# jmduarte/gnn-fpga

Hardware: AMD Instinct MI355X
Metric: edges/sec (EdgeNet+NodeNet fwd) on 100k-edge TrackML graphs; % HBM roofline (higher is better)
Workload: dtype f32; 1 GPU; c3 synthetic TrackML ACTS graphs: 256 graphs/launch/GPU x (10k hits, 100k segments), F=3, D=8, 3 MP iterations + final edge pass, index form resident in HBM; graphs_per_gpu=256, hits_per_graph=10000, segments_per_graph=100000

## Files before the change

### gnn-fpga_amd/csrc/sell_pipeline.hip

```cpp
#include "common.h"

#include <cstdlib>
#include <type_traits>

namespace {
using namespace gnn;

constexpr int SLICE = 16;
constexpr int DESC = 8;

template <int F, int D>
struct TL {
    static constexpr int d4 = D / 4, C = F + D;
    static constexpr int a4(int x) { return (x + 3) & ~3; }
    static constexpr int o_w2 = 0;
    static constexpr int o_in = a4(o_w2 + d4);
    static constexpr int in_sz = d4 + F * d4;
    static constexpr int o_4 = a4(o_in + in_sz);
    static constexpr int w4_sz = d4 + D * d4;
    static constexpr int o_m = a4(o_4 + w4_sz);
    static constexpr int m_sz = d4 + C * d4;
    static constexpr int m_st = a4(m_sz);
    static constexpr int o_b2 = o_m + 5 * m_st;
    static constexpr int used = o_b2 + 1;
// ... 1839 lines not shown
        }
        const int nq = (sg1 - sg0 + NTEAM - 1) / NTEAM;
        const int q0 = (((local - rot) % per_xcd) + per_xcd) % per_xcd;
        rot = (rot + nq) % per_xcd;
        for (int q = q0; SPLIT && sg0 + NTEAM * q < sg1; q += per_xcd) {
            const int sl = sg0 + NTEAM * q + team;
            if (sl >= sg1) continue;
            const int ib = __builtin_amdgcn_readfirstlane(in_off[sl]);
            const int il = (__builtin_amdgcn_readfirstlane(in_off[sl + 1]) - ib) >> 4;
            if (il <= 0) continue;
            const int i16 = 4 * mem + hs;
            const int64_t n = (int64_t)sl * SLICE + i16;
            float acc[DL], ownQ[DL];
            load_vec<DL>(U + n * D + DL * p, acc);
            load_own_w<D, EX>(QS, n, p, ownQ);
            sweep_w<D, XP, EX>(in_nbr + ib, i16, il, (int)n_pad, PR, p, ownQ, w2, b2, acc);
            store_vec<DL>(U + n * D + DL * p, acc);
        }
        if constexpr (SPLIT) {
            ++ngrp;
            if (lane == 0) bump(pha);
            for (int spins = 0; spins < kSpinLimit && ld(pha) < NSW * ngrp; ++spins) __builtin_amdgcn_s_sleep(2);
        }
        for (int q = q0; sg0 + NTEAM * q < sg1; q += per_xcd, seq += NTEAM) {
            const int sl = sg0 + NTEAM * q + team;
            const bool on = sl < sg1;
            float acc[DL];
            if (on) {
                const int ob = __builtin_amdgcn_readfirstlane(out_off[sl]);
                const int ol = (__builtin_amdgcn_readfirstlane(out_off[sl + 1]) - ob) >> 4;
                const int i16 = 4 * mem + hs;
                const int64_t n = (int64_t)sl * SLICE + i16;
                float ownP[DL];
                load_vec<DL>(U + n * D + DL * p, acc);
                if constexpr (!SPLIT) {
                    const int ib = __builtin_amdgcn_readfirstlane(in_off[sl]);
                    const int il = (__builtin_amdgcn_readfirstlane(in_off[sl + 1]) - ib) >> 4;
                    float ownQ[DL];
                    load_own_w<D, EX>(QS, n, p, ownQ);
                    load_own_w<D, EX>(PR, n, p, ownP);
                    sweep_w<D, XP, EX>(in_nbr + ib, i16, il, (int)n_pad, PR, p, ownQ, w2, b2, acc);
                } else {
                    load_own_w<D, EX>(PR, n, p, ownP);
                }
                sweep_w<D, XP, EX>(out_nbr + ob, i16, ol, (int)n_pad, QS, p, ownP, w2, b2, acc);
#pragma unroll
                for (int i = 0; i < DL; ++i) acc[i] = tanh_f(acc[i]);
            }
            const int slot = seq % NSLOT, gen = seq / NSLOT;
            for (int spins = 0; spins < kSpinLimit && ld(cons + slot) < gen; ++spins) __builtin_amdgcn_s_sleep(2);
            float *tr = ring + slot * 16 * B::tr_stride;
            if (on) {
                const int i16 = 4 * mem + hs;
                const int64_t n = (int64_t)sl * SLICE + i16;
                store_vec<DL>(tr + i16 * B::tr_stride + DL * p, acc);
                if (p < F) tr[i16 * B::tr_stride + D + p] = X[n * F + p];
            }
            if (mem == 0 && lane == 0) __hip_atomic_store(meta + slot, on ? sl : -1, __ATOMIC_RELAXED, __HIP_MEMORY_SCOPE_WORKGROUP);
            asm volatile("s_waitcnt lgkmcnt(0)" ::: "memory");
            if (lane == 0) bump(prod + slot);
        }
        if constexpr (!SPLIT) {
            ++ngrp;
            if (lane == 0) bump(pha);
            for (int spins = 0; spins < kSpinLimit && ld(pha) < NSW * ngrp; ++spins) __builtin_amdgcn_s_sleep(2);
        }
    }
    asm volatile("s_waitcnt lgkmcnt(0)" ::: "memory");
    if (lane == 0) bump(fin);
}

template <int F, int D>
struct MT {
    static_assert(D == 8, "fp32 matrix-core tables are laid out for D = 8");
    static constexpr int C = F + D;
    static constexpr bool PACK = F <= 4;
    static constexpr int NS = PACK ? 3 : F <= 8 ? 4 : 5;
    static constexpr int o_h0 = 0;
    static constexpr int o_t = 64;
    static constexpr int t_sz = NS * 64;
    static constexpr int o_w4 = o_t + 3 * t_sz;
    static constexpr int o_b = o_w4 + 128;
    static constexpr int total = o_b + 5 * 16;
    static constexpr int slot_k(int s, int g)
    {
        if (PACK) {
            if (g == 0) return s;
            if (g == 1) return 4 + s;
            if (g == 2) return s == 0 ? 3 : s == 1 ? 7 : (0 < F ? D : -1);
            return 1 + s < F ? D + 1 + s : -1;
        }
        if (s < 4) {
            if (g == 0) return s;
            if (g == 1) return 4 + s;
            const int xi = (g == 2) ? s : 4 + s;
            return xi < F ? D + xi : -1;
        }
        return 8 + g < F ? D + 8 + g : -1;
    }
};

template <int F, int D>
constexpr int mt_total()
{
    if constexpr (D == 8) return MT<F, D>::total;
    else return 0;
}

template <int F, int D>
__device__ __forceinline__ float mt_entry(const gnn_params_t &p, int i, bool last)
{
    using M = MT<F, D>;
    constexpr int C = F + D;
    if (i < 64) {
        const int row = i & 15, g = i >> 4;
        return (row < 8 && g < F && g < 4) ? p.Win[row * F + g] : 0.0f;
    }
    if (i < M::o_w4) {
        const int j = i - M::o_t, T = j / M::t_sz, st = (j % M::t_sz) >> 6, row = j & 15, g = (j >> 4) & 3;
        const int k = M::slot_k(st, g);
        if (k < 0) return 0.0f;
        if (last) {
            if (T > 0) return 0.0f;
            return kTwoLog2e * p.W1[(row & 7) * 2 * C + (row >> 3) * C + k];
        }
        if (T == 2) return row < 8 ? p.W3[row * 3 * C + 2 * C + k] : 0.0f;
        const int c = row >> 2, w = row & 3, d = 2 * c + (w & 1);
        return (w < 2) ? kTwoLog2e * p.W1[d * 2 * C + T * C + k] : p.W3[d * 3 * C + T * C + k];
    }
    if (i < M::o_b) {
        const int j = i - M::o_w4, st = j >> 6, row = j & 15, g = (j >> 4) & 3;
        return row < 8 ? p.W4[row * D + 2 * g + st] : 0.0f;
    }
    const int j = i - M::o_b, which = j >> 4, row = j & 15;
    switch (which) {
    case 0: return row < 8 ? p.bin[row] : 0.0f;
    case 1:
        if (last) return row < 8 ? kTwoLog2e * p.b1[row] : 0.0f;
        return (row & 3) < 2 ? kTwoLog2e * p.b1[2 * (row >> 2) + (row & 1)] : 0.0f;
    case 2: return 0.0f;
    case 3: return (!last && row < 8) ? p.b3[row] : 0.0f;
    default: return row < 8 ? p.b4[row] : 0.0f;
    }
}

template <int F, int D, bool LAST, bool XP, bool FIRST>
__global__ __launch_bounds__(1024) void k_iter2(
    const float *__restrict__ X, const float *__restrict__ table, gnn_params_t p,
    float *__restrict__ table_out,
    const int32_t *__restrict__ tiles, const int32_t *__restrict__ in_off,
    const int32_t *__restrict__ in_off16, const int32_t *__restrict__ in_nbr16,
    const int32_t *__restrict__ out_off, const int32_t *__restrict__ out_off16,
    const int32_t *__restrict__ out_nbr16, const int32_t *__restrict__ sched_a,
    const int32_t *__restrict__ sched_b, const float *__restrict__ PR,
    const float *__restrict__ QS, float *__restrict__ U, float *__restrict__ PRn,
    float *__restrict__ QSn, float *__restrict__ Pc, float *__restrict__ Qc, int64_t n_pad,
    int n_tiles, int capA, int capB, int xbuf_floats)
{
    using L = TL<F, D>;
    constexpr int d4 = L::d4, NT = 1024, NWV = NT / 64, NC = 3;
    extern __shared__ __attribute__((aligned(16))) float smem[];
    float *lds = smem, *bufA = smem + L::total, *bufB = bufA + (int64_t)capA * 2 * D;
    float *xbuf = bufB + (int64_t)capB * 2 * D;
    const int tid = threadIdx.x, lane = tid & 63, q = lane & 3, i16 = lane >> 2;
    const int wv = __builtin_amdgcn_readfirstlane(tid >> 6);
    if constexpr (FIRST) {
        for (int idx = tid; idx < L::total; idx += NT) {
            const float v = table_entry<F, D>(p, idx);
            lds[idx] = v;
            if (blockIdx.x == 0) table_out[idx] = v;
        }
        if (blockIdx.x == 0)
            write_null_rows<F, D, XP>(p, PRn, const_cast<float *>(PR), QSn, const_cast<float *>(QS),
                                      U, Pc, Qc, n_pad);
    } else {
        stage4<NT>(table, lds, L::total / 4);
    }
    float *mt = xbuf + (FIRST ? xbuf_floats : 0);
    if constexpr (D == 8)
        for (int i = tid; i < MT<F, D>::total; i += NT) mt[i] = mt_entry<F, D>(p, i, LAST);
    int tile = (gridDim.x & 7) ? (int)blockIdx.x
                               : (int)((blockIdx.x & 7) * (gridDim.x >> 3) + (blockIdx.x >> 3));
    if (tile >= n_tiles) return;

    struct Desc { int s_begin, s_end, in_lo, in_cnt, out_lo, out_cnt, sbase; };
    auto load_desc = [&](int t) {
        const int32_t *td = tiles + (int64_t)t * DESC;
        Desc d;
        d.s_begin = td[0]; d.s_end = td[1]; d.in_lo = td[2]; d.in_cnt = td[3];
        d.out_lo = td[4]; d.out_cnt = td[5]; d.sbase = td[7];
        return d;
    };
    auto slice_a = [&](const Desc &d, int r) { return sched_a[d.sbase + r * NWV + wv]; };

    auto stage_issue = [&](const float *src, float *buf, int nrec) {
        const int pieces = (nrec * 2 * D + 255) / 256;
        unsigned lb = (unsigned)lane * 16u;
        asm volatile("" : "+v"(lb));
        for (int c = wv; c < pieces; c += NWV)
            __builtin_amdgcn_global_load_lds(
                (const __attribute__((address_space(1))) void *)(
                    reinterpret_cast<const char *>(src + (int64_t)c * 256) + lb),
                (__attribute__((address_space(3))) void *)(buf + c * 256), 16, 0, 0);
    };
    auto put_null = [&](float *buf, int nrec, auto which) {
        constexpr int M = decltype(which)::value;
        const int pieces = (nrec * 2 * D + 255) / 256;
        if (wv == (pieces > 0 ? (pieces - 1) % NWV : 0) && lane < 4) {
            int l = lane;
            asm volatile("" : "+v"(l));
#pragma unroll
            for (int i = 0; i < d4; ++i) {
                float v = (M == 0) ? lds[l * L::stride + L::o_m + i] : 0.0f, z = 0.0f;
                if (XP) v = (M == 0) ? __builtin_amdgcn_exp2f(v) : 1.0f;
                asm volatile("" : "+v"(v), "+v"(z));
                buf[nrec * 2 * D + l * 2 * d4 + i] = v;
                buf[nrec * 2 * D + l * 2 * d4 + d4 + i] = z;
            }
        }
    };
    using WinA = std::integral_constant<int, 0>;
    using WinB = std::integral_constant<int, 1>;
    auto stage_commit = [&](float *buf, int nrec, auto which) {
        a_wait_all();
        put_null(buf, nrec, which);
    };

    auto x_image = [&](float *buf, int cap) { return buf + cap * 2 * D - (cap * F + 63) / 64 * 64; };
    auto xstage_issue = [&](int lo, int cnt, float *buf, int cap) {
        const int pieces = (cnt * F + 63) / 64;
        float *xb = x_image(buf, cap);
        unsigned lb = (unsigned)lane * 4u;
        asm volatile("" : "+v"(lb));
        for (int c = wv; c < pieces; c += NWV)
            __builtin_amdgcn_global_load_lds(
                (const __attribute__((address_space(1))) void *)(
                    reinterpret_cast<const char *>(X + (int64_t)lo * F + c * 64) + lb),
                (__attribute__((address_space(3))) void *)(xb + c * 64), 4, 0, 0);
    };
    auto h0_of = [&](const float *wl, const float *x, float *hn) {
        float hl[d4];
        role_gemv<d4, 0, F>(wl + L::o_in, x, x, hl);
#pragma unroll
        for (int i = 0; i < d4; ++i) hl[i] = tanh_f(hl[i]);
        quad_allgather<d4>(hl, hn);
    };
    auto compute_window = [&](float *buf, int cnt, int cap, auto which) {
        constexpr int M = decltype(which)::value;
        static_assert(2 * D * 4 - F * 4 >= 16, "a record must be longer than an X row (see x_image)");
        const float *xb = x_image(buf, cap);
        const int rounds = (cnt + NT / 4 - 1) / (NT / 4);
        const int x_off = (int)(xb - buf);
        auto round_fence = [&](int r) {
            if ((r + 1) * (NT / 4) * 2 * D > x_off) __syncthreads();
        };
        auto null_fence = [&]() {
            if ((cnt + 1) * 2 * D > x_off) __syncthreads();
        };
        a_wait_all();
        __syncthreads();
        if constexpr (D == 8) {
            typedef float f4v __attribute__((ext_vector_type(4)));
            using MTL = MT<F, D>;
            const float *mb = mt + MTL::o_b;
            const int hit = lane & 15, g = lane >> 4;
            const float a0 = mt[MTL::o_h0 + lane];
            static_assert(MTL::PACK, "the fused first launch exists for F <= 3 only");
            float ar[MTL::NS];
#pragma unroll
            for (int st = 0; st < MTL::NS; ++st) ar[st] = mt[MTL::o_t + MTL::t_sz * M + 64 * st + lane];
            const f4v bias0 = *reinterpret_cast<const f4v *>(mb + 4 * g);
            const f4v biasr = *reinterpret_cast<const f4v *>(mb + 16 + 16 * M + 4 * g);
            for (int r = 0; r < rounds; ++r) {
                const int h = (r * NWV + wv) * 16 + hit;
                const bool live = h < cnt;
                float xs[F];
#pragma unroll
                for (int k = 0; k < F; ++k) xs[k] = live ? xb[h * F + k] : 0.0f;
                round_fence(r);
                float b0 = 0.0f;
#pragma unroll
                for (int k = 0; k < F; ++k) b0 = (g == k) ? xs[k] : b0;
                f4v hq = __builtin_amdgcn_mfma_f32_16x16x4f32(a0, b0, bias0, 0, 0, 0);
                const float hh[4] = {tanh_f(hq.x), tanh_f(hq.y), tanh_f(hq.z), tanh_f(hq.w)};
                const float h3a = __int_as_float(__builtin_amdgcn_ds_bpermute(hit << 2, __float_as_int(hh[3])));
                const float h3b = __int_as_float(__builtin_amdgcn_ds_bpermute((16 + hit) << 2, __float_as_int(hh[3])));
                f4v c = biasr;
#pragma unroll
                for (int st = 0; st < MTL::NS; ++st) {
                    float b = hh[st];
                    if (g == 2) b = st == 0 ? h3a : st == 1 ? h3b : xs[0];
                    if (g == 3) b = 1 + st < F ? xs[1 + st < F ? 1 + st : 0] : 0.0f;
                    c = __builtin_amdgcn_mfma_f32_16x16x4f32(ar[st], b, c, 0, 0, 0);
                }
                if constexpr (XP) {
                    c.x = __builtin_amdgcn_exp2f(c.x);
                    c.y = __builtin_amdgcn_exp2f(c.y);
                }
                if (live) *reinterpret_cast<f4v *>(buf + h * 2 * D + 4 * g) = c;
            }
            null_fence();
            put_null(buf, cnt, which);
            return;
        }
        for (int r = 0; r < rounds; ++r) {
            const int h = r * (NT / 4) + (tid >> 2);
            const bool live = h < cnt;
            int woff = q * L::stride;
            asm volatile("" : "+v"(woff));
            const float *wl = lds + woff;
            float x[F], hn[D], rec[2 * d4];
#pragma unroll
            for (int k = 0; k < F; ++k) x[k] = live ? xb[h * F + k] : 0.0f;
            round_fence(r);
            if (!live) continue;
            h0_of(wl, x, hn);
            if constexpr (d4 == 2) {
                role_gemv_burst<D, F>(wl + L::o_m + (2 * M) * L::m_st, hn, x, rec);
                role_gemv_burst<D, F>(wl + L::o_m + (2 * M + 1) * L::m_st, hn, x, rec + d4);
            } else {
                role_gemv<d4, D, F>(wl + L::o_m + (2 * M) * L::m_st, hn, x, rec);
                role_gemv<d4, D, F>(wl + L::o_m + (2 * M + 1) * L::m_st, hn, x, rec + d4);
            }
            if constexpr (XP)
#pragma unroll
                for (int i = 0; i < d4; ++i) rec[i] = __builtin_amdgcn_exp2f(rec[i]);
            store_vec<2 * d4>(buf + h * 2 * D + q * 2 * d4, rec);
        }
        null_fence();
        put_null(buf, cnt, which);
    };

    struct PreA0 { int len; int c[NC]; AVec<d4> Q, U; };
    constexpr bool XPRE = F <= 4;
    struct PreB0 { int len; int c[NC]; AVec<d4> P; AVec<XPRE ? F : 0> x; };
    struct PreX { int len; int c[NC]; AVec<F> x; };
    using PreA = std::conditional_t<FIRST, PreX, PreA0>;
    using PreB = std::conditional_t<FIRST, PreX, PreB0>;
    const unsigned lo_list = (unsigned)(q * SLICE + i16) * 4u;
    const unsigned lo_rec = (unsigned)(i16 * 2 * D + q * 2 * d4) * 4u;
    const unsigned lo_vec = (unsigned)(i16 * D + q * d4) * 4u;
    const unsigned lo_x = (unsigned)(i16 * F) * 4u;
    auto prefetchA = [&](PreA &p, int slice_) {
        const int slice = __builtin_amdgcn_readfirstlane(slice_);
        p.len = (__builtin_amdgcn_readfirstlane(in_off[slice + 1]) -
                 __builtin_amdgcn_readfirstlane(in_off[slice])) >> 4;
        const int32_t *li = in_nbr16 + __builtin_amdgcn_readfirstlane(in_off16[slice]);
#define GNN_PF(C_) if (8 * C_ < p.len) a_load_i32_s<C_ * 4 * SLICE * 4>(p.c[C_], li, lo_list);
        GNN_PF(0) GNN_PF(1) GNN_PF(2)
#undef GNN_PF
        const int64_t n0 = (int64_t)slice * SLICE;
        if constexpr (FIRST) {
            p.x.load_s(X + n0 * F, lo_x);
        } else {
            p.Q.load_s(QS + n0 * 2 * D, lo_rec);
            p.U.load_s(U + n0 * D, lo_vec);
        }
    };
    auto prefetchB = [&](PreB &p, int slice_) {
        const int slice = __builtin_amdgcn_readfirstlane(slice_);
        p.len = (__builtin_amdgcn_readfirstlane(out_off[slice + 1]) -
                 __builtin_amdgcn_readfirstlane(out_off[slice])) >> 4;
        const int32_t *lo = out_nbr16 + __builtin_amdgcn_readfirstlane(out_off16[slice]);
#define GNN_PF(C_) if (8 * C_ < p.len) a_load_i32_s<C_ * 4 * SLICE * 4>(p.c[C_], lo, lo_list);
        GNN_PF(0) GNN_PF(1) GNN_PF(2)
#undef GNN_PF
        static_assert(NC == 3, "prefetch is written out for 3 words (24 steps)");
        const int64_t n0 = (int64_t)slice * SLICE;
        if constexpr (!FIRST) p.P.load_s(PR + n0 * 2 * D, lo_rec);
        if constexpr (XPRE || FIRST) p.x.load_s(X + n0 * F, lo_x);
    };
    auto arriveA = [&](PreA &p) {
        a_wait_all();
        a_fence(p.c);
        if constexpr (FIRST) {
            p.x.fence();
        } else {
            p.Q.fence();
            p.U.fence();
        }
    };
    auto arriveB = [&](PreB &p) {
        a_wait_all();
        a_fence(p.c);
        if constexpr (!FIRST) p.P.fence();
        if constexpr (XPRE || FIRST) p.x.fence();
    };

    constexpr int MAXR = 5;
    float ac0[d4], ac1[d4], ac2[d4], ac3[d4], ac4[d4];
    auto acc_put = [&](int r, const float *a) {
#pragma unroll
        for (int i = 0; i < d4; ++i) {
            ac0[i] = (r == 0) ? a[i] : ac0[i];
            ac1[i] = (r == 1) ? a[i] : ac1[i];
            ac2[i] = (r == 2) ? a[i] : ac2[i];
            ac3[i] = (r == 3) ? a[i] : ac3[i];
            ac4[i] = (r >= 4) ? a[i] : ac4[i];
        }
    };
    auto acc_get = [&](int r, float *a) {
#pragma unroll
        for (int i = 0; i < d4; ++i)
            a[i] = (r == 0) ? ac0[i] : (r == 1) ? ac1[i] : (r == 2) ? ac2[i] : (r == 3) ? ac3[i] : ac4[i];
    };
    static_assert(MAXR == 5, "accumulator slots are written out for 5 rounds");
#pragma unroll
    for (int i = 0; i < d4; ++i) ac0[i] = ac1[i] = ac2[i] = ac3[i] = ac4[i] = 0.0f;

    Desc d = load_desc(tile);
    PreA a_cur, a_nxt;
    PreB b_cur, b_nxt;
    if constexpr (FIRST) {
        xstage_issue(d.in_lo, d.in_cnt, bufA, capA);
        if (slice_a(d, 0) >= 0) prefetchA(a_cur, slice_a(d, 0));
        compute_window(bufA, d.in_cnt, capA, WinA{});
    } else {
        stage_issue(PR + (int64_t)d.in_lo * 2 * D, bufA, d.in_cnt);
        if (slice_a(d, 0) >= 0) prefetchA(a_cur, slice_a(d, 0));
        __syncthreads();
        stage_commit(bufA, d.in_cnt, WinA{});
    }
    if (slice_a(d, 0) >= 0) arriveA(a_cur);

    float w2[d4];
    for (;;) {
        __syncthreads();
#pragma unroll
        for (int i = 0; i < d4; ++i) w2[i] = lds[q * L::stride + L::o_w2 + i];
        const float b2 = lds[L::o_b2];
        const int rounds = (d.s_end - d.s_begin + NWV - 1) / NWV;
        if constexpr (FIRST)
            xstage_issue(d.out_lo, d.out_cnt, bufB, capB);
        else
            stage_issue(QS + (int64_t)d.out_lo * 2 * D, bufB, d.out_cnt);
        auto roundA = [&](int r, auto lr) {
            constexpr bool LR = decltype(lr)::value;
            const int slice = slice_a(d, r);
            const int next = LR ? -1 : slice_a(d, r + 1);
            if constexpr (LR) {
                if (slice_a(d, 0) >= 0) prefetchB(b_cur, slice_a(d, 0));
            } else {
                if (next >= 0) prefetchA(a_nxt, next);
            }
            float acc[d4];
            if (slice >= 0) {
                float Qn[d4];
                if constexpr (FIRST) {
                    int woff = q * L::stride;
                    asm volatile("" : "+v"(woff));
                    const float *wl = lds + woff;
                    float xo[F], h0[D];
                    a_cur.x.get(xo);
                    h0_of(wl, xo, h0);
                    role_gemv<d4, D, F>(wl + L::o_m + 2 * L::m_st, h0, xo, Qn);
                    if constexpr (XP)
#pragma unroll
                        for (int i = 0; i < d4; ++i) Qn[i] = __builtin_amdgcn_exp2f(Qn[i]);
                    role_gemv<d4, D, F>(wl + L::o_m + 4 * L::m_st, h0, xo, acc);
                } else {
                    a_cur.U.get(acc);
                    a_cur.Q.get(Qn);
                }
                const int len = __builtin_amdgcn_readfirstlane(a_cur.len);
                sweep16<D, NC, XP, !FIRST>(a_cur.c, in_nbr16, in_off16, slice, i16, len, bufA, q, Qn, w2, b2, acc);
            }
            if constexpr (!LR) {
                if (next >= 0) {
                    arriveA(a_nxt);
                    a_cur = a_nxt;
                }
            }
            if (slice >= 0) acc_put(r, acc);
        };
        for (int r = 0; r + 1 < rounds; ++r) roundA(r, std::false_type{});
        roundA(rounds - 1, std::true_type{});
        if constexpr (FIRST)
            compute_window(bufB, d.out_cnt, capB, WinB{});
        else
            stage_commit(bufB, d.out_cnt, WinB{});
        if (slice_a(d, 0) >= 0) arriveB(b_cur);
        __syncthreads();
        const int tnext = tile + gridDim.x;
        Desc dn = d;
        if (tnext < n_tiles) {
            dn = load_desc(tnext);
            if constexpr (FIRST)
                xstage_issue(dn.in_lo, dn.in_cnt, bufA, capA);
            else
                stage_issue(PR + (int64_t)dn.in_lo * 2 * D, bufA, dn.in_cnt);
        }
        auto roundB = [&](int r, auto lr) {
            constexpr bool LR = decltype(lr)::value;
            const int slice = slice_a(d, r);
            const int next = LR ? -1 : slice_a(d, r + 1);
            if constexpr (LR) {
                if (tnext < n_tiles && slice_a(dn, 0) >= 0) prefetchA(a_cur, slice_a(dn, 0));
            } else {
                if (next >= 0) prefetchB(b_nxt, next);
            }
            float xv[F], acc[d4];
            if (slice >= 0) {
                float Pn[d4];
                acc_get(r, acc);
                if constexpr (XPRE || FIRST) {
                    b_cur.x.get(xv);
                } else {
                    const float *xr = X + ((int64_t)__builtin_amdgcn_readfirstlane(slice) * SLICE + i16) * F;
#pragma unroll
                    for (int k = 0; k < F; ++k) xv[k] = xr[k];
                }
                if constexpr (FIRST) {
                    int woff = q * L::stride;
                    asm volatile("" : "+v"(woff));
                    const float *wl = lds + woff;
                    float h0[D];
                    h0_of(wl, xv, h0);
                    role_gemv<d4, D, F>(wl + L::o_m + 0 * L::m_st, h0, xv, Pn);
                    if constexpr (XP)
#pragma unroll
                        for (int i = 0; i < d4; ++i) Pn[i] = __builtin_amdgcn_exp2f(Pn[i]);
                } else {
                    b_cur.P.get(Pn);
                }
                const int len = __builtin_amdgcn_readfirstlane(b_cur.len);
                sweep16<D, NC, XP, false>(b_cur.c, out_nbr16, out_off16, slice, i16, len, bufB, q, Pn, w2, b2, acc);
            }
            if constexpr (!LR) {
                if (next >= 0) {
                    arriveB(b_nxt);
                    b_cur = b_nxt;
                }
            }
            if constexpr (D == 8) {
                if (slice >= 0) {
                    using MTL = MT<F, D>;
                    typedef float f4v __attribute__((ext_vector_type(4)));
                    const float *mb = mt + MTL::o_b;
                    const int hit = lane & 15, g = lane >> 4;
                    const int from = ((hit << 2) | g) << 2;
                    const float q0 = __int_as_float(__builtin_amdgcn_ds_bpermute(from, __float_as_int(tanh_f(acc[0]))));
                    const float q1 = __int_as_float(__builtin_amdgcn_ds_bpermute(from, __float_as_int(tanh_f(acc[1]))));
                    float xm[F];
#pragma unroll
                    for (int k = 0; k < F; ++k)
                        xm[k] = __int_as_float(__builtin_amdgcn_ds_bpermute(hit << 4, __float_as_int(xv[k])));
                    f4v h = *reinterpret_cast<const f4v *>(mb + 64 + 4 * g);
                    h = __builtin_amdgcn_mfma_f32_16x16x4f32(mt[MTL::o_w4 + lane], q0, h, 0, 0, 0);
                    h = __builtin_amdgcn_mfma_f32_16x16x4f32(mt[MTL::o_w4 + 64 + lane], q1, h, 0, 0, 0);
                    const float hh[4] = {tanh_f(h.x), tanh_f(h.y), tanh_f(h.z), tanh_f(h.w)};
                    float h3a = 0.0f, h3b = 0.0f;
                    if constexpr (MTL::PACK) {
                        h3a = __int_as_float(__builtin_amdgcn_ds_bpermute(hit << 2, __float_as_int(hh[3])));
                        h3b = __int_as_float(__builtin_amdgcn_ds_bpermute((16 + hit) << 2, __float_as_int(hh[3])));
                    }
                    auto slot_in = [&](int st) {
                        if constexpr (MTL::PACK) {
                            if (g < 2) return hh[st];
                            if (g == 2) return st == 0 ? h3a : st == 1 ? h3b : (0 < F ? xm[0] : 0.0f);
                            float v = 0.0f;
#pragma unroll
                            for (int k = 1; k < F; ++k) v = (k == 1 + st) ? xm[k] : v;
                            return v;
                        }
                        if (st < 4) {
                            if (g < 2) return hh[st];
                            float v = 0.0f;
#pragma unroll
                            for (int k = 0; k < F; ++k)
                                if (k == st || k == 4 + st) v = (g == (k < 4 ? 2 : 3) && (k & 3) == st) ? xm[k] : v;
                            return v;
                        }
                        float v = 0.0f;
#pragma unroll
                        for (int k = 8; k < F; ++k) v = (g == k - 8) ? xm[k] : v;
                        return v;
                    };
                    float bin_[MTL::NS];
#pragma unroll
                    for (int st = 0; st < MTL::NS; ++st) bin_[st] = slot_in(st);
                    const int64_t n = (int64_t)__builtin_amdgcn_readfirstlane(slice) * SLICE + hit;
                    constexpr int NP = LAST ? 1 : 3;
#pragma unroll
                    for (int T = 0; T < NP; ++T) {
                        f4v c = *reinterpret_cast<const f4v *>(mb + 16 * (1 + T) + 4 * g);
#pragma unroll
                        for (int st = 0; st < MTL::NS; ++st)
                            c = __builtin_amdgcn_mfma_f32_16x16x4f32(mt[MTL::o_t + MTL::t_sz * T + 64 * st + lane],
                                                                     bin_[st], c, 0, 0, 0);
                        if constexpr (LAST) {
                            if constexpr (XP) {
                                c.x = __builtin_amdgcn_exp2f(c.x); c.y = __builtin_amdgcn_exp2f(c.y);
                                c.z = __builtin_amdgcn_exp2f(c.z); c.w = __builtin_amdgcn_exp2f(c.w);
                            }
                            *reinterpret_cast<f4v *>((g < 2 ? Pc : Qc) + n * D + 4 * (g & 1)) = c;
                        } else if (T < 2) {
                            if constexpr (XP) {
                                c.x = __builtin_amdgcn_exp2f(c.x);
                                c.y = __builtin_amdgcn_exp2f(c.y);
                            }
                            *reinterpret_cast<f4v *>((T == 0 ? PRn : QSn) + n * 2 * D + 4 * g) = c;
                        } else if (g < 2) {
                            *reinterpret_cast<f4v *>(U + n * D + 4 * g) = c;
                        }
                    }
                }
            } else if (slice >= 0) {
                int woff = q * L::stride;
                asm volatile("" : "+v"(woff));
                const float *wl = lds + woff;
                float ql[d4], qa[D], hl[d4], hn[D];
#pragma unroll
                for (int i = 0; i < d4; ++i) ql[i] = tanh_f(acc[i]);
                quad_allgather<d4>(ql, qa);
                role_gemv<d4, D, 0>(wl + L::o_4, qa, qa, hl);
#pragma unroll
                for (int i = 0; i < d4; ++i) hl[i] = tanh_f(hl[i]);
                quad_allgather<d4>(hl, hn);
                const int64_t n0 = (int64_t)__builtin_amdgcn_readfirstlane(slice) * SLICE;
                auto at = [](float *base, unsigned off) {
                    return reinterpret_cast<float *>(reinterpret_cast<char *>(base) + off);
                };
                if constexpr (LAST)
                    emit_to<F, D, LAST, XP>(wl, hn, xv, at(Pc + n0 * D, lo_vec), at(Qc + n0 * D, lo_vec), nullptr);
                else
                    emit_to<F, D, LAST, XP>(wl, hn, xv, at(PRn + n0 * 2 * D, lo_rec), at(QSn + n0 * 2 * D, lo_rec),
                                            at(U + n0 * D, lo_vec));
            }
        };
        for (int r = 0; r + 1 < rounds; ++r) roundB(r, std::false_type{});
        roundB(rounds - 1, std::true_type{});
        if (tnext >= n_tiles) break;
        if constexpr (FIRST)
            compute_window(bufA, dn.in_cnt, capA, WinA{});
        else
            stage_commit(bufA, dn.in_cnt, WinA{});
        if (slice_a(dn, 0) >= 0) arriveA(a_cur);
        tile = tnext;
        d = dn;
    }
}

template <int F, int D, bool XP>
__global__ __launch_bounds__((Cfg<F, D>::NT)) void k_edge(
    const int32_t *__restrict__ chunks, const int32_t *__restrict__ src,
    const int32_t *__restrict__ dst, const int32_t *__restrict__ sd16,
    const float *__restrict__ Pc, const float *__restrict__ Qc,
    const float *__restrict__ table, float *__restrict__ e, int64_t n_pad, int chunks_per_xcd,
    int n_chunks)
{
    using G = Cfg<F, D>;
    const float *__restrict__ W2 = table + TL<F, D>::o_flat;
    constexpr int NT = G::NT;
    extern __shared__ __attribute__((aligned(16))) float win[];
    const int chunk = (blockIdx.x & 7) * chunks_per_xcd + (blockIdx.x >> 3);
    if (chunk >= n_chunks) return;
    const int32_t *cd = chunks + (int64_t)chunk * DESC;
    const int e0 = cd[0], e1 = cd[1], s_lo = cd[2], s_cnt = cd[3], d_lo = cd[4], d_cnt = cd[5],
              mode = cd[6];
    float *winA = win, *winB = win + (s_cnt + 1) * D;
    if (G::ed_rec > 0 && mode) {
        stage4<NT>(Pc + (int64_t)s_lo * D, winA, s_cnt * D / 4);
        stage4<NT>(Pc + n_pad * D, winA + s_cnt * D, D / 4);
        stage4<NT>(Qc + (int64_t)d_lo * D, winB, d_cnt * D / 4);
        stage4<NT>(Qc + n_pad * D, winB + d_cnt * D, D / 4);
        __syncthreads();
    }
    const float b2 = W2[D];
    auto score = [&](const float *p, const float *qq) {
        float acc = b2;
#pragma unroll
        for (int k = 0; k < D; ++k)
            acc = fmaf(W2[k], XP ? __builtin_amdgcn_rcpf(fmaf(p[k], qq[k], 1.0f)) : r_f(p[k] + qq[k]), acc);
        return r_f(acc);
    };
    if (G::ed_rec > 0 && mode) {
        constexpr int B8 = 8;
        for (int j0 = e0 + (int)threadIdx.x; j0 < e1; j0 += B8 * NT) {
            unsigned w[B8];
#pragma unroll
            for (int u = 0; u < B8; ++u) w[u] = (j0 + u * NT < e1) ? (unsigned)sd16[j0 + u * NT] : 0u;
#pragma unroll
            for (int u = 0; u < B8; ++u) {
                if (j0 + u * NT < e1) {
                    float p[D], qq[D];
                    load_vec<D>(winA + (w[u] & 0xFFFFu) * D, p);
                    load_vec<D>(winB + (w[u] >> 16) * D, qq);
                    e[j0 + u * NT] = score(p, qq);
                }
            }
        }
    } else {
        for (int j = e0 + (int)threadIdx.x; j < e1; j += NT) {
            float p[D], qq[D];
            const int s = src[j], d = dst[j];
            load_vec<D>(Pc + (int64_t)s * D, p);
            load_vec<D>(Qc + (int64_t)d * D, qq);
            e[j] = score(p, qq);
        }
    }
}

template <int F, int D, bool XP>
__global__ __launch_bounds__(256) void k_edge_tw(const int32_t *__restrict__ src, const int32_t *__restrict__ dst,
                                                 const float *__restrict__ Pc, const float *__restrict__ Qc,
                                                 const float *__restrict__ table, float *__restrict__ e, int64_t n_pad,
                                                 int64_t n_segments)
{
    const float *__restrict__ W2 = table + TL<F, D>::o_flat;
    const int64_t j = xcd_block() * 256 + threadIdx.x;
    if (j >= n_segments) return;
    int s = src[j], d = dst[j];
    if (s < 0) s = d = (int)n_pad;
    float p[D], qq[D];
    load_vec<D>(Pc + (int64_t)s * D, p);
// ... 72 lines not shown
    w.table = take((size_t)table_floats);
    w.PRa = take(rec); w.PRb = take(rec); w.QSa = take(rec); w.QSb = take(rec);
    w.U = take(vec); w.Pc = take(vec); w.Qc = take(vec);
    w.t16 = reinterpret_cast<unsigned *>(take((size_t)t16_words));
    w.bytes = off;
    return w;
}

template <int F, int D>
constexpr int t16_words()
{
    if constexpr (D % 32 == 0 && F <= 4) return BL<F, D>::total > BX<F, D>::total ? BL<F, D>::total : BX<F, D>::total;
    else if constexpr (D % 32 == 0 && F <= 8) return BL<F, D>::total;
    else if constexpr (D % 16 == 0 && F <= 4) return BX<F, D>::total;
    else return 0;
}
template <int F, int D>
constexpr bool can_exact_wide() { return D % 16 == 0 && F <= 4; }
constexpr int64_t kRoleSplitMinHits = 32768;

inline int wide_window_records(int row_bytes)
{
    static const long kb = getenv("GNN_WIDE_WINDOW_KB") ? atol(getenv("GNN_WIDE_WINDOW_KB")) : 3072;
    const long r = kb * 1024 / row_bytes;
    return (int)(r < 0 ? 0 : r > 0x3FFFFFFF ? 0x3FFFFFFF : r);
}

template <int F, int D, bool XP>
int forward_t(const gnn_plan_t *pl, const gnn_params_t *p, int n_iters, float *e_out, char *ws,
              hipStream_t s)
{
    using L = TL<F, D>;
    using G = Cfg<F, D>;
    const int64_t Np = pl->n_pad, E = pl->n_segments;
    Ws w = carve(ws, Np, L::total, D, t16_words<F, D>());
    constexpr bool can_bf = D % 32 == 0 && F <= 8;
    const bool bf = can_bf && (p->flags & GNN_FLAG_BF16_MLP) && n_iters > 0 &&
                    (uint64_t)(Np + 2) * D * 4 < (1ull << 32);
    if constexpr (can_bf)
        if (bf && Np > 0)
            GNN_LAUNCH("k_pack16", (k_pack16<F, D>), 64, 256, s, *p, w.t16, w.PRa, w.PRb, w.QSa, w.QSb, Np,
                       XP ? 1 : 0);
    constexpr bool can_ex = can_exact_wide<F, D>();
    const bool ex = can_ex && !bf && n_iters > 0 && Np > 0 && (uint64_t)(Np + 2) * D * 8 < (1ull << 32) &&
                    !getenv("GNN_NO_WIDE_EXACT");
    if (Np == 0 || G::pack_first || ex)
        GNN_LAUNCH("k_pack", (k_pack<F, D, XP>), (L::total + 255) / 256, 256, s, *p, w.table, w.PRa, w.PRb,
                   w.QSa, w.QSb, w.U, w.Pc, w.Qc, Np);
    if constexpr (can_ex)
        if (ex)
            GNN_LAUNCH("k_pack32", (k_pack32<F, D>), 64, 256, s, *p, reinterpret_cast<float *>(w.t16), w.PRa, w.PRb,
                       w.QSa, w.QSb, Np, XP ? 1 : 0);
    float *PR = w.PRa, *PRn = w.PRb, *QS = w.QSa, *QSn = w.QSb;
    if (Np > 0) {
        const int nt = (int)pl->n_tiles;
        const int tpx = (nt + 7) / 8;
        const size_t it_lds = (size_t)(L::total + (G::it_rec > 0 ? pl->iter_lds_records : 0) * 2 * D + 4) * sizeof(float);
        static DevOnce attr_done;
        if (attr_done.need()) {
            (void)hipFuncSetAttribute(reinterpret_cast<const void *>(&k_iter<F, D, true, XP>), hipFuncAttributeMaxDynamicSharedMemorySize, G::lds_bytes);
            (void)hipFuncSetAttribute(reinterpret_cast<const void *>(&k_iter<F, D, false, XP>), hipFuncAttributeMaxDynamicSharedMemorySize, G::lds_bytes);
        }
#ifdef GNN_DIAG
        const char *ab = getenv("GNN_ABLATE");
        const int ablate = ab ? atoi(ab) : 0;
#else
        const int ablate = 0;
#endif
        bool use2 = false, fuse_first = false;
        size_t it2_lds = 0, it2_lds_first = 0;
        int capA = 0, capB = 0, grid2 = 0, xbuf_floats = 0;
        if constexpr (G::iter2) {
            const int64_t rpp = 128 / D;
            const int64_t capa = (pl->iter_lds_in + rpp - 1) / rpp * rpp + rpp;
            const int64_t capb = (pl->iter_lds_out + rpp - 1) / rpp * rpp + rpp;
            use2 = !getenv("GNN_NO_ITER2") && nt > 0 && pl->n_lds_tiles == nt &&
                   pl->in_nbr16 && pl->out_nbr16 && pl->in_off16 && pl->out_off16 && pl->sched_a && pl->sched_b;
            capA = (int)capa;
            capB = (int)capb;
            constexpr int mt_floats = mt_total<F, D>();
            it2_lds = (size_t)(L::total + (capa + capb) * 2 * D + 4 + mt_floats) * sizeof(float);
            if (it2_lds > (size_t)G::lds_bytes) use2 = false;
            xbuf_floats = 0;
            it2_lds_first = it2_lds;
            fuse_first = G::fuse_first && XP && use2 && n_iters >= 2 && it2_lds_first <= (size_t)G::lds_bytes &&
                         !getenv("GNN_NO_FUSE_FIRST");
            const int n_cu = device_cus();
            static DevOnce it2_attr;
            if (it2_attr.need()) {
                (void)hipFuncSetAttribute(reinterpret_cast<const void *>(&k_iter2<F, D, true, XP, false>), hipFuncAttributeMaxDynamicSharedMemorySize, G::lds_bytes);
                (void)hipFuncSetAttribute(reinterpret_cast<const void *>(&k_iter2<F, D, false, XP, false>), hipFuncAttributeMaxDynamicSharedMemorySize, G::lds_bytes);
                if constexpr (XP && G::fuse_first)
                    (void)hipFuncSetAttribute(reinterpret_cast<const void *>(&k_iter2<F, D, false, true, true>), hipFuncAttributeMaxDynamicSharedMemorySize, G::lds_bytes);
            }
            grid2 = nt < n_cu ? nt : n_cu;
        }
        bool input_done = false;
        if constexpr (can_bf) {
            if (bf && G::pack_first) {
                using B = BL<F, D>;
                const size_t lds_in = (size_t)(B::template tm_words<false>() + 5 * D + 4 * 16 * B::tr_stride) * 4;
                static DevOnce in_attr;
                if (in_attr.need())
                    (void)hipFuncSetAttribute(reinterpret_cast<const void *>(&k_input4_bf<F, D, false, XP>), hipFuncAttributeMaxDynamicSharedMemorySize, G::lds_bytes);
                const int64_t g_need = (Np * 4 + 255) / 256;
                GNN_LAUNCH_SH("k_input4", (k_input4_bf<F, D, false, XP>), (unsigned)(g_need < 512 ? g_need : 512), 256,
                              lds_in, s, pl->X, w.table, w.t16, PR, QS, w.U, w.Pc, w.Qc, Np);
                input_done = true;
            }
        }
        if constexpr (can_ex) {
            if (ex) {
                using B = BX<F, D>;
                const size_t lds_in = (size_t)(B::template tm_words<false>() + 5 * D + 16 * 16 * B::tr_stride) * 4;
                static DevOnce inx_attr;
                if (inx_attr.need())
                    (void)hipFuncSetAttribute(reinterpret_cast<const void *>(&k_input4_x<F, D, false, XP>), hipFuncAttributeMaxDynamicSharedMemorySize, G::lds_bytes);
                const int64_t g_need = (Np * 4 + 1023) / 1024;
                const int64_t g_cap = device_cus();
                GNN_LAUNCH_SH("k_input4", (k_input4_x<F, D, false, XP>), (unsigned)(g_need < g_cap ? g_need : g_cap), 1024,
                              lds_in, s, pl->X, w.table, reinterpret_cast<const float *>(w.t16), PR, QS, w.U, w.Pc, w.Qc, Np);
                input_done = true;
            }
        }
        if (!fuse_first && !input_done) {
            const int64_t g_need = (Np * 4 + 255) / 256;
            const unsigned g = (unsigned)(g_need < 4096 ? g_need : 4096);
            if (n_iters == 0)
                GNN_LAUNCH("k_input4", (k_input4<F, D, true, XP>), g, 256, s, pl->X, *p, w.table, PR, QS,
                           PRn, QSn, w.U, w.Pc, w.Qc, Np);
            else
                GNN_LAUNCH("k_input4", (k_input4<F, D, false, XP>), g, 256, s, pl->X, *p, w.table, PR, QS,
                           PRn, QSn, w.U, w.Pc, w.Qc, Np);
        }
        for (int t = 0; t < n_iters; ++t) {
            if constexpr (G::iter2) {
                if (use2) {
#define GNN_IT2(LAST_, FIRST_, LDS_)                                                                   \
    GNN_LAUNCH_SH("k_iter2", (k_iter2<F, D, LAST_, XP, FIRST_>), grid2, 1024, LDS_, s, pl->X, w.table, *p, \
                  w.table, pl->tiles, pl->in_off, pl->in_off16, pl->in_nbr16, pl->out_off,             \
                  pl->out_off16, pl->out_nbr16, pl->sched_a, pl->sched_b, PR, QS, w.U, PRn, QSn, w.Pc,  \
                  w.Qc, Np, nt, capA, capB, xbuf_floats)
                    if (XP && t == 0 && fuse_first) {
                        if constexpr (XP && G::fuse_first) GNN_IT2(false, true, it2_lds_first);
                    } else if (t + 1 == n_iters)
                        GNN_IT2(true, false, it2_lds);
                    else
                        GNN_IT2(false, false, it2_lds);
#undef GNN_IT2
                    float *t1 = PR; PR = PRn; PRn = t1;
                    float *t2 = QS; QS = QSn; QSn = t2;
                    continue;
                }
            }
            bool launched = false;
            if constexpr (can_bf) {
                if (bf) {
                    using B = BL<F, D>;
                    static DevOnce bf_attr;
                    if (bf_attr.need()) {
                        (void)hipFuncSetAttribute(reinterpret_cast<const void *>(&k_iter_w<F, D, true, XP>), hipFuncAttributeMaxDynamicSharedMemorySize, G::lds_bytes);
                        (void)hipFuncSetAttribute(reinterpret_cast<const void *>(&k_iter_w<F, D, false, XP>), hipFuncAttributeMaxDynamicSharedMemorySize, G::lds_bytes);
                    }
                    const int ncu = device_cus();
                    const unsigned wgs = (unsigned)(((nt < ncu ? nt : ncu) + 7) / 8 * 8);
                    const size_t trw = (size_t)2 * 4 * 16 * B::tr_stride + 4;
                    const int wmax = wide_window_records(4 * D);
// ... 277 lines not shown
```

Measured before the change: 30.44 billion edges/s.

## Compute own-slice P/Q/U via MFMA in fused first iteration instead of per-lane LDS

In the fused first-iteration kernel, each tile now runs an own_pass that recomputes the input MLP for its own slices on matrix cores and writes P, Q and U to global memory. The main rounds then prefetch those values like later iterations do, instead of recomputing them from X with per-lane LDS weight reads. The aim is to replace scalar recomputation in the hot sweep with batched MFMA work. In exchange it adds an extra global write and read round trip per tile, a barrier, and more LDS for the new coefficient table. It also drops the cross-tile prefetch of the next tile's first slice.

```diff
diff --git a/gnn-fpga_amd/csrc/sell_pipeline.hip b/gnn-fpga_amd/csrc/sell_pipeline.hip
--- a/gnn-fpga_amd/csrc/sell_pipeline.hip
+++ b/gnn-fpga_amd/csrc/sell_pipeline.hip
@@ -1945,6 +1945,9 @@
     static constexpr int o_w4 = o_t + 3 * t_sz;
     static constexpr int o_b = o_w4 + 128;
     static constexpr int total = o_b + 5 * 16;
+    static constexpr int o_c = total;
+    static constexpr int o_cb = o_c + t_sz;
+    static constexpr int total_first = o_cb + 16;
     static constexpr int slot_k(int s, int g)
     {
         if (PACK) {
@@ -1967,6 +1970,13 @@
 constexpr int mt_total()
 {
     if constexpr (D == 8) return MT<F, D>::total;
+    else return 0;
+}
+
+template <int F, int D>
+constexpr int mt_total_first()
+{
+    if constexpr (D == 8) return MT<F, D>::total_first;
     else return 0;
 }
 
@@ -2028,20 +2038,26 @@
     const int tid = threadIdx.x, lane = tid & 63, q = lane & 3, i16 = lane >> 2;
     const int wv = __builtin_amdgcn_readfirstlane(tid >> 6);
     if constexpr (FIRST) {
+        if (blockIdx.x == 0)
+            write_null_rows<F, D, XP>(p, PRn, const_cast<float *>(PR), QSn, const_cast<float *>(QS),
+                                      U, Pc, Qc, n_pad);
         for (int idx = tid; idx < L::total; idx += NT) {
             const float v = table_entry<F, D>(p, idx);
             lds[idx] = v;
             if (blockIdx.x == 0) table_out[idx] = v;
         }
-        if (blockIdx.x == 0)
-            write_null_rows<F, D, XP>(p, PRn, const_cast<float *>(PR), QSn, const_cast<float *>(QS),
-                                      U, Pc, Qc, n_pad);
     } else {
         stage4<NT>(table, lds, L::total / 4);
     }
     float *mt = xbuf + (FIRST ? xbuf_floats : 0);
     if constexpr (D == 8)
         for (int i = tid; i < MT<F, D>::total; i += NT) mt[i] = mt_entry<F, D>(p, i, LAST);
+    constexpr bool OWN = FIRST && D == 8;
+    if constexpr (OWN) {
+        using MTL = MT<F, D>;
+        for (int i = tid; i < MTL::t_sz + 16; i += NT)
+            mt[MTL::o_c + i] = mt_entry<F, D>(p, i < MTL::t_sz ? MTL::o_t + i : MTL::o_b + 16 + (i - MTL::t_sz), true);
+    }
     int tile = (gridDim.x & 7) ? (int)blockIdx.x
                                : (int)((blockIdx.x & 7) * (gridDim.x >> 3) + (blockIdx.x >> 3));
     if (tile >= n_tiles) return;
@@ -2126,12 +2142,14 @@
             typedef float f4v __attribute__((ext_vector_type(4)));
             using MTL = MT<F, D>;
             const float *mb = mt + MTL::o_b;
-            const int hit = lane & 15, g = lane >> 4;
-            const float a0 = mt[MTL::o_h0 + lane];
+            int l = lane;
+            asm volatile("" : "+v"(l));
+            const int hit = l & 15, g = l >> 4;
+            const float a0 = mt[MTL::o_h0 + l];
             static_assert(MTL::PACK, "the fused first launch exists for F <= 3 only");
             float ar[MTL::NS];
 #pragma unroll
-            for (int st = 0; st < MTL::NS; ++st) ar[st] = mt[MTL::o_t + MTL::t_sz * M + 64 * st + lane];
+            for (int st = 0; st < MTL::NS; ++st) ar[st] = mt[MTL::o_t + MTL::t_sz * M + 64 * st + l];
             const f4v bias0 = *reinterpret_cast<const f4v *>(mb + 4 * g);
             const f4v biasr = *reinterpret_cast<const f4v *>(mb + 16 + 16 * M + 4 * g);
             for (int r = 0; r < rounds; ++r) {
@@ -2198,8 +2216,8 @@
     constexpr bool XPRE = F <= 4;
     struct PreB0 { int len; int c[NC]; AVec<d4> P; AVec<XPRE ? F : 0> x; };
     struct PreX { int len; int c[NC]; AVec<F> x; };
-    using PreA = std::conditional_t<FIRST, PreX, PreA0>;
-    using PreB = std::conditional_t<FIRST, PreX, PreB0>;
+    using PreA = std::conditional_t<FIRST && !OWN, PreX, PreA0>;
+    using PreB = std::conditional_t<FIRST && !OWN, PreX, PreB0>;
     const unsigned lo_list = (unsigned)(q * SLICE + i16) * 4u;
     const unsigned lo_rec = (unsigned)(i16 * 2 * D + q * 2 * d4) * 4u;
     const unsigned lo_vec = (unsigned)(i16 * D + q * d4) * 4u;
@@ -2213,7 +2231,10 @@
         GNN_PF(0) GNN_PF(1) GNN_PF(2)
 #undef GNN_PF
         const int64_t n0 = (int64_t)slice * SLICE;
-        if constexpr (FIRST) {
+        if constexpr (OWN) {
+            p.Q.load_s(Qc + n0 * D, lo_vec);
+            p.U.load_s(U + n0 * D, lo_vec);
+        } else if constexpr (FIRST) {
             p.x.load_s(X + n0 * F, lo_x);
         } else {
             p.Q.load_s(QS + n0 * 2 * D, lo_rec);
@@ -2230,13 +2251,14 @@
 #undef GNN_PF
         static_assert(NC == 3, "prefetch is written out for 3 words (24 steps)");
         const int64_t n0 = (int64_t)slice * SLICE;
-        if constexpr (!FIRST) p.P.load_s(PR + n0 * 2 * D, lo_rec);
+        if constexpr (OWN) p.P.load_s(Pc + n0 * D, lo_vec);
+        else if constexpr (!FIRST) p.P.load_s(PR + n0 * 2 * D, lo_rec);
         if constexpr (XPRE || FIRST) p.x.load_s(X + n0 * F, lo_x);
     };
     auto arriveA = [&](PreA &p) {
         a_wait_all();
         a_fence(p.c);
-        if constexpr (FIRST) {
+        if constexpr (FIRST && !OWN) {
             p.x.fence();
         } else {
             p.Q.fence();
@@ -2246,11 +2268,71 @@
     auto arriveB = [&](PreB &p) {
         a_wait_all();
         a_fence(p.c);
-        if constexpr (!FIRST) p.P.fence();
+        if constexpr (!FIRST || OWN) p.P.fence();
         if constexpr (XPRE || FIRST) p.x.fence();
     };
 
     constexpr int MAXR = 5;
+    auto own_pass = [&](const Desc &dd) {
+        if constexpr (OWN) {
+            typedef float f4v __attribute__((ext_vector_type(4)));
+            using MTL = MT<F, D>;
+            static_assert(MTL::PACK, "the fused first launch exists for F <= 3 only");
+            const int nr = (dd.s_end - dd.s_begin + NWV - 1) / NWV;
+            int l = lane;
+            asm volatile("" : "+v"(l));
+            const int hit = l & 15, g = l >> 4;
+            int sl[MAXR];
+            float xs[MAXR][F];
+#pragma unroll
+            for (int r = 0; r < MAXR; ++r) {
+                sl[r] = r < nr ? __builtin_amdgcn_readfirstlane(slice_a(dd, r)) : -1;
+                if (sl[r] >= 0) {
+                    const float *xr = X + ((int64_t)sl[r] * SLICE + hit) * F;
+#pragma unroll
+                    for (int k = 0; k < F; ++k) xs[r][k] = xr[k];
+                }
+            }
+            const float *mb = mt + MTL::o_b;
+            const float a0 = mt[MTL::o_h0 + l];
+            float apq[MTL::NS], au[MTL::NS];
+#pragma unroll
+            for (int st = 0; st < MTL::NS; ++st) {
+                apq[st] = mt[MTL::o_c + 64 * st + l];
+                au[st] = mt[MTL::o_t + MTL::t_sz * 2 + 64 * st + l];
+            }
+            const f4v bias0 = *reinterpret_cast<const f4v *>(mb + 4 * g);
+            const f4v biaspq = *reinterpret_cast<const f4v *>(mt + MTL::o_cb + 4 * g);
+            const f4v biasu = *reinterpret_cast<const f4v *>(mb + 16 * 3 + 4 * g);
+#pragma unroll
+            for (int r = 0; r < MAXR; ++r) {
+                if (sl[r] < 0) continue;
+                float b0 = 0.0f;
+#pragma unroll
+                for (int k = 0; k < F; ++k) b0 = (g == k) ? xs[r][k] : b0;
+                const f4v hq = __builtin_amdgcn_mfma_f32_16x16x4f32(a0, b0, bias0, 0, 0, 0);
+                const float hh[4] = {tanh_f(hq.x), tanh_f(hq.y), tanh_f(hq.z), tanh_f(hq.w)};
+                const float h3a = __int_as_float(__builtin_amdgcn_ds_bpermute(hit << 2, __float_as_int(hh[3])));
+                const float h3b = __int_as_float(__builtin_amdgcn_ds_bpermute((16 + hit) << 2, __float_as_int(hh[3])));
+                f4v c = biaspq, u = biasu;
+#pragma unroll
+                for (int st = 0; st < MTL::NS; ++st) {
+                    float b = hh[st];
+                    if (g == 2) b = st == 0 ? h3a : st == 1 ? h3b : xs[r][0];
+                    if (g == 3) b = 1 + st < F ? xs[r][1 + st < F ? 1 + st : 0] : 0.0f;
+                    c = __builtin_amdgcn_mfma_f32_16x16x4f32(apq[st], b, c, 0, 0, 0);
+                    u = __builtin_amdgcn_mfma_f32_16x16x4f32(au[st], b, u, 0, 0, 0);
+                }
+                c.x = __builtin_amdgcn_exp2f(c.x); c.y = __builtin_amdgcn_exp2f(c.y);
+                c.z = __builtin_amdgcn_exp2f(c.z); c.w = __builtin_amdgcn_exp2f(c.w);
+                const int64_t n = (int64_t)sl[r] * SLICE + hit;
+                *reinterpret_cast<f4v *>((g < 2 ? Pc : Qc) + n * D + 4 * (g & 1)) = c;
+                if (g < 2) *reinterpret_cast<f4v *>(U + n * D + 4 * g) = u;
+            }
+            a_wait_all();
+        }
+    };
+
     float ac0[d4], ac1[d4], ac2[d4], ac3[d4], ac4[d4];
     auto acc_put = [&](int r, const float *a) {
 #pragma unroll
@@ -2276,6 +2358,10 @@
     PreB b_cur, b_nxt;
     if constexpr (FIRST) {
         xstage_issue(d.in_lo, d.in_cnt, bufA, capA);
+        if constexpr (OWN) {
+            __syncthreads();
+            own_pass(d);
+        }
         if (slice_a(d, 0) >= 0) prefetchA(a_cur, slice_a(d, 0));
         compute_window(bufA, d.in_cnt, capA, WinA{});
     } else {
@@ -2309,7 +2395,7 @@
             float acc[d4];
             if (slice >= 0) {
                 float Qn[d4];
-                if constexpr (FIRST) {
+                if constexpr (FIRST && !OWN) {
                     int woff = q * L::stride;
                     asm volatile("" : "+v"(woff));
                     const float *wl = lds + woff;
@@ -2326,7 +2412,7 @@
                     a_cur.Q.get(Qn);
                 }
                 const int len = __builtin_amdgcn_readfirstlane(a_cur.len);
-                sweep16<D, NC, XP, !FIRST>(a_cur.c, in_nbr16, in_off16, slice, i16, len, bufA, q, Qn, w2, b2, acc);
+                sweep16<D, NC, XP, !FIRST || OWN>(a_cur.c, in_nbr16, in_off16, slice, i16, len, bufA, q, Qn, w2, b2, acc);
             }
             if constexpr (!LR) {
                 if (next >= 0) {
@@ -2358,7 +2444,8 @@
             const int slice = slice_a(d, r);
             const int next = LR ? -1 : slice_a(d, r + 1);
             if constexpr (LR) {
-                if (tnext < n_tiles && slice_a(dn, 0) >= 0) prefetchA(a_cur, slice_a(dn, 0));
+                if constexpr (!OWN)
+                    if (tnext < n_tiles && slice_a(dn, 0) >= 0) prefetchA(a_cur, slice_a(dn, 0));
             } else {
                 if (next >= 0) prefetchB(b_nxt, next);
             }
@@ -2373,7 +2460,7 @@
 #pragma unroll
                     for (int k = 0; k < F; ++k) xv[k] = xr[k];
                 }
-                if constexpr (FIRST) {
+                if constexpr (FIRST && !OWN) {
                     int woff = q * L::stride;
                     asm volatile("" : "+v"(woff));
                     const float *wl = lds + woff;
@@ -2494,6 +2581,10 @@
         for (int r = 0; r + 1 < rounds; ++r) roundB(r, std::false_type{});
         roundB(rounds - 1, std::true_type{});
         if (tnext >= n_tiles) break;
+        if constexpr (OWN) {
+            own_pass(dn);
+            if (slice_a(dn, 0) >= 0) prefetchA(a_cur, slice_a(dn, 0));
+        }
         if constexpr (FIRST)
             compute_window(bufA, dn.in_cnt, capA, WinA{});
         else
@@ -2732,7 +2823,7 @@
             it2_lds = (size_t)(L::total + (capa + capb) * 2 * D + 4 + mt_floats) * sizeof(float);
             if (it2_lds > (size_t)G::lds_bytes) use2 = false;
             xbuf_floats = 0;
-            it2_lds_first = it2_lds;
+            it2_lds_first = it2_lds + (size_t)(mt_total_first<F, D>() - mt_floats) * sizeof(float);
             fuse_first = G::fuse_first && XP && use2 && n_iters >= 2 && it2_lds_first <= (size_t)G::lds_bytes &&
                          !getenv("GNN_NO_FUSE_FIRST");
             const int n_cu = device_cus();
```

Result: slower. 29.57 billion edges/s (-2.9%).
